# AIflowerQ/InvPref_KDD_2022

Measured on AMD Instinct MI355X. Metric: training interactions/sec, Yahoo-implicit InvPref, higher is better.
Workload: dtype f32; 1 GPU; yahoo_r3_implicit_shaped; users=15400, items=1000, envs=4, factor_num=64, scaling=strong, interactions_total=250154, global_batch=8192, interactions_per_gpu=250154, batch_per_gpu=8192, estep_every_steps=155, parallelism=single GPU

## Files before the change

### invpref_kdd_2022_amd/csrc/invpref_plan.cpp

```cpp
#include "../../include/invpref_plan.h"

#include <algorithm>
#include <atomic>
#include <cstdlib>
#include <cmath>
#include <cstring>
#include <exception>
#include <memory>
#include <mutex>
#include <thread>
#include <vector>

struct InvPrefHostPlan {
    std::vector<int32_t> arr[8];
    std::unique_ptr<int32_t[]> big[8];
    size_t big_n[8] = {0, 0, 0, 0, 0, 0, 0, 0};
    int32_t *alloc(int which, size_t n) {
        big[which].reset(new int32_t[n ? n : 1]);
        big_n[which] = n;
        return big[which].get();
    }
};

namespace {
// ... 263 lines not shown
    for (int c = 0; c < ncls; c++) {
        n_ur[(size_t)c] = (int32_t)cit[(size_t)(2 * c)].size();
        n_ir[(size_t)c] = (int32_t)cit[(size_t)(2 * c + 1)].size();
        uit.insert(uit.end(), cit[(size_t)(2 * c)].begin(), cit[(size_t)(2 * c)].end());
        const std::vector<int32_t> &rows = srows[(size_t)c];
        int64_t k = (int64_t)std::nearbyint(p.stream_split * (double)rows.size());
        if (p.fill_cap) {
            const int64_t room = p.fill_cap / ncls - cdiv(n_ur[(size_t)c], p.rounds_per_task);
            k = std::min<int64_t>((int64_t)rows.size(), std::max<int64_t>(k, room * p.rows_per_stream_task));
        }
        k = std::max<int64_t>(0, std::min<int64_t>(k, (int64_t)rows.size()));
        for (int li = 0; li < 2; li++) {
            const int64_t a = li == 0 ? 0 : k, b = li == 0 ? k : (int64_t)rows.size();
            std::vector<int32_t> &dst = li == 0 ? s1[(size_t)c] : s2[(size_t)c];
            for (int64_t q = a; q < b; q++)
                if (rows[(size_t)q] & kItemBit) dst.push_back(rows[(size_t)q]);
            for (int64_t q = a; q < b; q++)
                if (!(rows[(size_t)q] & kItemBit)) dst.push_back(rows[(size_t)q]);
        }
    }
    for (int c = 0; c < ncls; c++) {
        cls[c][0] = ub; cls[c][1] = n_ur[(size_t)c]; ub += n_ur[(size_t)c];
        cls[c][4] = ib; cls[c][5] = n_ir[(size_t)c]; ib += n_ir[(size_t)c];
    }
    int32_t sb = 0;
    for (int c = 0; c < ncls; c++) { cls[c][2] = sb; cls[c][3] = (int32_t)s1[(size_t)c].size(); sb += cls[c][3]; }
    for (int c = 0; c < ncls; c++) { cls[c][6] = sb; cls[c][7] = (int32_t)s2[(size_t)c].size(); sb += cls[c][7]; }
    {
        std::vector<size_t> off((size_t)(2 * ncls));
        size_t tot[2] = {0, 0};
        for (int q = 0; q < 2 * ncls; q++) { off[(size_t)q] = tot[q & 1]; tot[q & 1] += cd[(size_t)q].size(); }
        int32_t *const dst[2] = {hp->alloc(0, tot[0]), hp->alloc(1, tot[1])};
        parallel_for(2 * ncls, nt, [&](int q) {
            if (!cd[(size_t)q].empty()) std::memcpy(dst[q & 1] + off[(size_t)q], cd[(size_t)q].data(), cd[(size_t)q].size() * 4);
            std::vector<int32_t>().swap(cd[(size_t)q]);
        });
    }
    for (int c = 0; c < ncls; c++) sr.insert(sr.end(), s1[(size_t)c].begin(), s1[(size_t)c].end());
    for (int c = 0; c < ncls; c++) sr.insert(sr.end(), s2[(size_t)c].begin(), s2[(size_t)c].end());
    hp->arr[7].assign(&cls[0][0], &cls[0][0] + 64);
    return hp;
}

InvPrefHostPlan *build_alt(const int64_t *cu, const int64_t *ci, const float *cy, int64_t n, const int64_t *pu, const int64_t *pi,
                           int64_t n_prev, int64_t U, int64_t I, const InvPrefAltPlanParams &p) {
    const bool has_cur = n > 0, has_prev = pu != nullptr && n_prev >= 0;
    if (U <= 0 || I <= 0 || n < 0 || (p.side != 0 && p.side != 1) || p.per_slice < 1 || p.n_classes < 1 || p.n_classes > 8 ||
        p.pend_job_min < 1 || p.pend_per_slice < 1 || (p.slots != 16 && p.slots != 32) || (has_cur && (!cu || !ci || !cy)) || (has_prev && (!pu || !pi)))
        return nullptr;
    const int ng = p.slots;
    const int ncls = p.n_classes;
    const int64_t own_num = p.side == 0 ? U : I, oth_num = p.side == 0 ? I : U;
    const int64_t *own = p.side == 0 ? cu : ci, *oth = p.side == 0 ? ci : cu, *ownp = p.side == 0 ? pu : pi;
    InvPrefHostPlan *hp = new InvPrefHostPlan();
    std::vector<int32_t> &lst = hp->arr[2], &ps = hp->arr[3];
    Side S, T, Sp;
    lst.assign((size_t)n * 4, 0);
    ps.assign((size_t)n, 0);
    bool ok = sort_side(own, n, own_num, S, 1, [&](int64_t i, int64_t j) {
        int32_t *d = lst.data() + (size_t)j * 4;
        d[0] = (int32_t)oth[i];
        d[1] = (int32_t)i;
        std::memcpy(d + 2, cy + i, 4);
    });
    ok = ok && sort_side(oth, n, oth_num, T, 1, [&](int64_t i, int64_t j) { ps[(size_t)i] = (int32_t)j; });
    ok = ok && sort_side(ownp, has_prev ? n_prev : 0, own_num, Sp, 1, [&](int64_t, int64_t) {});
    if (!ok) {
        delete hp;
        return nullptr;
    }
    std::vector<int32_t> &desc = hp->arr[0], &pend = hp->arr[1], &stream = hp->arr[4];
    int32_t cls[8][4];
    std::memset(cls, 0, sizeof(cls));
    int32_t rb = 0;
    std::vector<std::vector<int32_t>> srows((size_t)ncls);
    for (int c = 0; c < ncls; c++) {
        std::vector<int32_t> arows, jrows;
        for (int64_t r = 0; r < own_num; r++) {
            if ((r >> kClassShift) % ncls != c) continue;
            if (S.cnt[(size_t)r] > 0) arows.push_back((int32_t)r);
            else if (Sp.cnt[(size_t)r] >= p.pend_job_min) jrows.push_back((int32_t)r);
            else srows[(size_t)c].push_back((int32_t)r);
        }
        std::vector<int32_t> d, it;
        if (has_cur) side_rounds(S, n, lst.data(), 4, 3, ng, p.per_slice, 1, 2, arows, d, it);
        const size_t n_a = d.size() / ((size_t)ng * 8);
        if (!jrows.empty()) side_rounds(Sp, 0, nullptr, 0, 0, ng, p.pend_per_slice, 1, 0, jrows, d, it);
        const size_t nr = d.size() / ((size_t)ng * 8);
        const size_t pbase = pend.size();
        pend.resize(pbase + nr * ng * 4, 0);
        for (size_t r = 0; r < nr; r++) {
            bool any = false;
            for (int sl = 0; sl < ng; sl++) {
                int32_t *dd = d.data() + (r * ng + sl) * 8, *pp = pend.data() + pbase + (r * ng + sl) * 4;
                const int64_t row = dd[0];
                if (row < 0) continue;
                const int gf = (dd[1] >> 1) & 31, g = gf ? gf : 32, k = sl % g;
                const int64_t cp = Sp.cnt[(size_t)row], p0 = Sp.ptr[(size_t)row];
                const int64_t ln = cdiv(cp, g);
                pp[0] = (int32_t)(p0 + std::min<int64_t>(k * ln, cp));
                pp[1] = (int32_t)(p0 + std::min<int64_t>((k + 1) * ln, cp));
                pp[2] = (int32_t)cp;
                any = any || cp > 0;
                if (r >= n_a) {
                    dd[1] &= 0x3f;
                    for (int q = 2; q < 8; q++) dd[q] = 0;
                }
            }
            if (any)
                for (int sl = 0; sl < ng; sl++) d[(r * ng + sl) * 8 + 1] |= (int32_t)0x80000000u;
        }
        desc.insert(desc.end(), d.begin(), d.end());
        cls[c][0] = rb;
        cls[c][1] = (int32_t)nr;
        rb += (int32_t)nr;
    }
    int32_t sb = 0;
    for (int c = 0; c < ncls; c++) {
        cls[c][2] = sb;
        cls[c][3] = (int32_t)srows[(size_t)c].size();
        sb += cls[c][3];
        for (int32_t r : srows[(size_t)c]) {
            const int32_t e[4] = {r, (int32_t)Sp.ptr[(size_t)r], (int32_t)Sp.ptr[(size_t)r + 1], (int32_t)Sp.cnt[(size_t)r]};
            stream.insert(stream.end(), e, e + 4);
        }
    }
    hp->arr[5].assign(&cls[0][0], &cls[0][0] + 32);
    return hp;
}

}

extern "C" {

static InvPrefHostPlan *build_alt_guarded(const int64_t *cu, const int64_t *ci, const float *cy, int64_t n, const int64_t *pu,
                                          const int64_t *pi, int64_t n_prev, int64_t U, int64_t I, const InvPrefAltPlanParams *p) {
    if (!p) return nullptr;
    try {
        return build_alt(cu, ci, cy, n, pu, pi, n_prev, U, I, *p);
    } catch (...) {
        return nullptr;
    }
}

InvPrefHostPlan *invpref_alt_plan_build(const int64_t *cur_users, const int64_t *cur_items, const float *cur_scores, int64_t n,
                                        const int64_t *prev_users, const int64_t *prev_items, int64_t n_prev,
                                        int64_t user_num, int64_t item_num, const InvPrefAltPlanParams *params) {
    return build_alt_guarded(cur_users, cur_items, cur_scores, n, prev_users, prev_items, n_prev, user_num, item_num, params);
}

int invpref_alt_plan_build_many(const int64_t *users, const int64_t *items, const float *scores, const int64_t *cur_lo,
                                const int64_t *cur_n, const int64_t *prev_lo, const int64_t *prev_n, const int32_t *side,
                                int32_t count, int64_t user_num, int64_t item_num, const InvPrefAltPlanParams *params,
                                InvPrefHostPlan **out, int32_t n_threads) {
    if (!users || !items || !scores || !cur_lo || !cur_n || !prev_lo || !prev_n || !side || !params || !out || count < 0) return -1;
    int nt = n_threads > 0 ? n_threads : (int)std::min<unsigned>(kMaxThreads, std::max(1u, std::thread::hardware_concurrency()));
    nt = std::max(1, std::min(nt, (int)count));
    std::atomic<int> next{0};
    auto work = [&]() {
        for (;;) {
            const int k = next.fetch_add(1);
            if (k >= count) return;
            InvPrefAltPlanParams p = *params;
            p.side = side[k];
            const bool hp = prev_n[k] >= 0;
            out[k] = build_alt_guarded(users + cur_lo[k], items + cur_lo[k], scores + cur_lo[k], cur_n[k],
// ... 100 lines not shown
```

### invpref_kdd_2022_amd/csrc/step_alt.hpp

```cpp

#ifdef ALT_STAMPS
#define ASTAMP(i) STAMP(i)
#else
#define ASTAMP(i) do { } while (0)
#endif

struct AltArgs {
    float *own_p[2];
    float *own_m[2], *own_v[2];
    const float *oth_p[2];
    float *Ev, *W, *b;
    float *mEv, *mW, *mb, *vEv, *vW, *vb;
    int E, D;
    const int4 *desc;
    const int4 *pend;
    const int4 *list;
    const int *push_slot;
    const int4 *stream;
    int rounds_per_task, rows_per_stream_task, n_cls;
    int cls[8][4];
    const int64_t *envs;
    const float *weights;
    StepScalars k;
    float r2_prev, r1_prev;
// ... 122 lines not shown
    if (lane < EMAX) scw[lane] = x.cw;
}
__device__ __forceinline__ void alt_stage_plain(const AltArgs &a, float *sEv, float *sW, float *sb, float *scw, bool pure) {
    constexpr int EMAX = 4, DP = 64;
    const int lane = threadIdx.x & 63;
    bool on[4], onb;
    alt_stage_lanes(a, lane, on, onb);
#pragma unroll
    for (int i = 0; i < 4; i++) {
        const int idx = lane + 64 * i, e = idx / DP, d = idx - e * DP;
        const bool o = on[i] && !pure;
        sEv[idx] = o ? a.Ev[e * a.D + d] : 0.f;
        sW[idx] = o ? a.W[e * a.D + d] : 0.f;
    }
    if (lane < EMAX) sb[lane] = (onb && !pure) ? a.b[lane] : 0.f;
    if (lane < EMAX) scw[lane] = ((a.flags & INVPREF_WEIGHTS_BY_ENV) && onb && !pure) ? a.weights[lane] : 1.f;
}

template <int THREADS>
struct AltGeo {
    static constexpr int NG = THREADS / 16, WAVES = THREADS / 64, DP = 64, EMAX = 4;
    static constexpr int SLAB = 2 * EMAX * DP + EMAX + kLossSlots;
    static constexpr int sEv = 0, sW = sEv + EMAX * DP, sb = sW + EMAX * DP;
    static constexpr int scw = sb + EMAX;
    static constexpr int mv = scw + EMAX;
    static constexpr int red = mv + WAVES * 4 * 64 * 4;
    static constexpr int total = red + NG * SLAB;
};

__device__ __forceinline__ void adam4_prev(float4 &p, float4 g, float4 &m, float4 &v, const AdamScalars &ad, float2 prev2) {
    AdamScalars ap = ad;
    ap.step_size = prev2.x; ap.bc2_sqrt = prev2.y;
    adam4(p, g, m, v, ap);
}

template <bool VEC, bool FULL, int MODE, int THREADS>
__device__ __forceinline__ void alt_task(const AltArgs &a, int r0, int slab_index, float *lds,
                                         const AdamScalars &ad_cur, float2 prev2, const StepScalars &k, int gen) {
    constexpr int LG = 16, EMAX = 4, UE = 2;
    using G = AltGeo<THREADS>;
    using L = AltGeo<THREADS>;
    static_assert(EvalLds<16, 4>::total == AltGeo<256>::total, "alt_task: the smallest-instance layout");
    constexpr int NG = G::NG, DP = G::DP;
    float *sEv = lds + L::sEv, *sW = lds + L::sW, *sb = lds + L::sb, *scw = lds + L::scw;
    float4 *mv = reinterpret_cast<float4 *>(lds + L::mv);
    float *red = lds + L::red;
    const int lg = threadIdx.x & (LG - 1), grp = threadIdx.x / LG, wave = threadIdx.x >> 6, lane = threadIdx.x & 63;
    float4 *mv_wave = mv + wave * 4 * 64;
    const bool implicit = a.flags & INVPREF_IMPLICIT;
    const bool rw_rec = a.flags & INVPREF_REWEIGHT_REC, rw_cls = a.flags & INVPREF_REWEIGHT_CLS;
    const bool by_env = a.flags & INVPREF_WEIGHTS_BY_ENV;
    const bool reg_env = a.flags & INVPREF_REG_ENV_EMBED;
    const bool pure = a.flags & INVPREF_PURE_MF;
    const bool dense = (a.flags & INVPREF_DENSE_REG) && !(a.flags & INVPREF_REG_ONLY_EMBED) && !pure;
    constexpr bool has_prev = MODE & 1, has_cur = MODE & 2;
    const int D = a.D;
    float *own0 = a.own_p[0], *own1 = a.own_p[1];
    const float *oth0 = a.oth_p[0], *oth1 = a.oth_p[1];

    ASTAMP(0);
    int4 d = a.desc[(r0 * NG + grp) * 2], d1 = a.desc[(r0 * NG + grp) * 2 + 1];
    int4 pd = make_int4(0, 0, 0, 0);
    if (has_prev) pd = a.pend[r0 * NG + grp];
    ASTAMP(1);
    float accLi = 0.f, accLe = 0.f, accLc = 0.f, accL2 = 0.f, accL1 = 0.f;
    float *slab = a.slabs + (int64_t)slab_index * G::SLAB;
    auto slot_of = [&](int g) {
        constexpr int GW = 64 / LG;
        return lds + L::mv + (g / GW) * (4 * 64 * 4) + (g % GW) * 2 * DP;
    };

    {
        constexpr int nr = 1;
        const int r = r0;
        const int4 dd = d, dd1 = d1;
        const int4 pdd = pd;
        const int row = dd.x, meta = dd.y;
        const bool active = row >= 0, leader = meta & 1;
        const int slices_f = (meta >> 1) & 31, mode = (meta >> 6) & 7;
        const int slices = slices_f ? slices_f : 32;
        const bool rpend = has_prev && (meta < 0);
        const int cnt_i = (meta >> 9) & 0x3fffff;
        const int nsmp = (active && has_cur) ? (mode == 7 ? dd.w - dd.z : mode) : 0;
        if (r == r0 + STAMP_ROUND) ASTAMP(2);
        const int s_lo = dd.z, s_hi1 = max(dd.w - 1, dd.z);
        const int *dwords = reinterpret_cast<const int *>(a.desc + (r * NG + grp) * 2);
        auto sample_at = [&](int sidx) {
            USample sm;
            if (FULL) {
                const int *src = mode == 7 ? reinterpret_cast<const int *>(a.list + min(s_lo + sidx, s_hi1)) : dwords + 2 + 3 * min(sidx, 1);
                sm.oth = src[0]; sm.ps = src[1]; sm.y = __builtin_bit_cast(float, src[2]);
            } else if (mode == 7) {
                const int4 q = a.list[dd.z + sidx];
                sm.oth = q.x; sm.ps = q.y; sm.y = __builtin_bit_cast(float, q.z);
            } else if (sidx == 0) { sm.oth = dd.z; sm.ps = dd.w; sm.y = __builtin_bit_cast(float, dd1.x); }
            else { sm.oth = dd1.y; sm.ps = dd1.z; sm.y = __builtin_bit_cast(float, dd1.w); }
            return sm;
        };
        const int rowc = active ? row : 0;
        float4 oi = row4<VEC, FULL>(own0, rowc, D, lg), oe = f4zero();
        float4 mi = row4<VEC, FULL>(a.own_m[0], rowc, D, lg), vi = row4<VEC, FULL>(a.own_v[0], rowc, D, lg);
        float4 me = f4zero(), ve = f4zero();
        if (!pure) {
            oe = row4<VEC, FULL>(own1, rowc, D, lg);
            me = row4<VEC, FULL>(a.own_m[1], rowc, D, lg); ve = row4<VEC, FULL>(a.own_v[1], rowc, D, lg);
        }
        constexpr int PB = kAltPendBatch;
        static_assert(PB * 2 * 64 * 4 <= 4 * G::SLAB && (4 * G::SLAB) % 4 == 0 && G::red % 4 == 0, "landing block: the wave's four slab rows");
        const int npend = (active && has_prev) ? pdd.y - pdd.x : 0;
        const float *pbase = a.pend_rows + (unsigned)(npend > 0 ? pdd.x : 0) * (unsigned)(2 * DP) + lg * 4;
        float *land = red + wave * 4 * G::SLAB;
        auto pland = [&](int s0) {
#pragma unroll
            for (int j = 0; j < PB; j++) {
                if (s0 + j < npend) {
                    const float *p = pbase + (unsigned)(s0 + j) * (unsigned)(2 * DP);
                    __builtin_amdgcn_global_load_lds((const __attribute__((address_space(1))) void *)p,
                                                     (__attribute__((address_space(3))) void *)(land + (2 * j) * 256), 16, 0, 0);
                    if (!pure)
                        __builtin_amdgcn_global_load_lds((const __attribute__((address_space(1))) void *)(p + DP),
                                                         (__attribute__((address_space(3))) void *)(land + (2 * j + 1) * 256), 16, 0, 0);
                }
            }
        };
        float4 gpi = f4zero(), gpe = f4zero();
        int n_wave = 0;
        if (rpend) {
            n_wave = npend;
#pragma unroll
            for (int g = 0; g < 64 / LG; g++) n_wave = max(n_wave, __builtin_amdgcn_readlane(npend, g * LG));
            pland(0);
        }

        struct Slot {
            float4 qi, qa;
            USample sm;
            int e, cs;
            float w;
        };
        Slot sl[UE];
        USample idn[UE];
        auto gather = [&](Slot &q, const USample &sm) {
            q.sm = sm;
            q.qi = row4<VEC, FULL>(oth0, sm.oth, D, lg);
            if (FULL) {
                const unsigned pso = (unsigned)sm.ps;
                if (!pure) {
                    q.qa = row4<VEC, FULL>(oth1, sm.oth, D, lg);
                    q.e = *reinterpret_cast<const int *>(reinterpret_cast<const char *>(a.envs) + pso * 8u);
                }
                if ((rw_rec || rw_cls) && !by_env) q.w = *reinterpret_cast<const float *>(reinterpret_cast<const char *>(a.weights) + pso * 4u);
                q.cs = *reinterpret_cast<const int *>(reinterpret_cast<const char *>(a.push_slot) + pso * 4u);
                return;
            }
            if (!pure) {
                q.qa = row4<VEC, FULL>(oth1, sm.oth, D, lg);
                q.e = (int)a.envs[sm.ps];
            }
            if ((rw_rec || rw_cls) && !by_env) q.w = a.weights[sm.ps];
            q.cs = a.push_slot[sm.ps];
        };
#pragma unroll
        for (int j = 0; j < UE; j++) {
            sl[j].qi = sl[j].qa = f4zero();
            sl[j].sm = USample{0, 0, 0.f};
            sl[j].e = sl[j].cs = 0;
            sl[j].w = 1.f;
            idn[j] = USample{0, 0, 0.f};
        }
        USample ls[2 * UE];
#pragma unroll
        for (int j = 0; j < 2 * UE; j++) ls[j] = USample{0, 0, 0.f};
        if (has_cur) {
            if (FULL) {
                if (__builtin_amdgcn_ballot_w64(mode == 7) != 0) {
#pragma unroll
                    for (int j = 0; j < 2 * UE; j++) {
                        const int4 q = a.list[mode == 7 ? min(s_lo + j, s_hi1) : 0];
                        ls[j] = USample{q.x, q.y, __builtin_bit_cast(float, q.z)};
                    }
                }
            } else {
#pragma unroll
                for (int j = 0; j < 2 * UE; j++)
                    if (j < nsmp) ls[j] = sample_at(j);
            }
        }
        auto psum = [&](int s0) {
            asm volatile("s_waitcnt vmcnt(0)" ::: "memory");
            float4 xi[PB], xe[PB];
#pragma unroll
            for (int j = 0; j < PB; j++) {
                xi[j] = *reinterpret_cast<const float4 *>(land + (2 * j) * 256 + lane * 4);
                xe[j] = pure ? f4zero() : *reinterpret_cast<const float4 *>(land + (2 * j + 1) * 256 + lane * 4);
            }
#pragma unroll
            for (int j = 0; j < PB; j++) {
                const bool has = s0 + j < npend;
                f4add(gpi, has ? xi[j] : f4zero());
                if (!pure) f4add(gpe, has ? xe[j] : f4zero());
            }
            if (s0 + PB < n_wave) pland(s0 + PB);
        };
        if (n_wave > 0) psum(0);
        if (has_cur) {
#pragma unroll
            for (int j = 0; j < UE; j++) {
                if (FULL) {
                    USample sm = ls[j];
                    if (mode != 7) sm = j == 0 ? USample{dd.z, dd.w, __builtin_bit_cast(float, dd1.x)} : USample{dd1.y, dd1.z, __builtin_bit_cast(float, dd1.w)};
                    if (mode == 0 || !active) sm = USample{0, 0, 0.f};
                    gather(sl[j], sm);
                } else if (j < nsmp) {
                    gather(sl[j], ls[j]);
                }
                idn[j] = ls[UE + j];
            }
        }
        AltStage stg;
#pragma unroll
        for (int i = 0; i < 9; i++) stg.g[i] = 0ull;
        stg.cw = 1.f;
        if (has_prev) {
            if (rpend) {
                for (int s0 = PB; s0 < n_wave; s0 += PB) psum(s0);
                if (slices > 1) {
                    float *mine = slot_of(grp);
                    *reinterpret_cast<float4 *>(mine + lg * 4) = gpi;
                    *reinterpret_cast<float4 *>(mine + DP + lg * 4) = gpe;
                    __syncthreads();
                    const int lead = grp & ~(slices - 1);
                    if (VEC && slices >= 8) {
                        if (active && leader) {
                            gpi = gpe = f4zero();
#pragma nounroll
                            for (int s = 0; s < slices; s += 8) {
                                float4 xi[8], xe[8];
                                const float *s8 = slot_of(lead + s) + lg * 4;
#pragma unroll
                                for (int j = 0; j < 8; j++) {
                                    xi[j] = *reinterpret_cast<const float4 *>(s8 + (j / 4) * (4 * 64 * 4) + (j % 4) * 2 * DP);
                                    xe[j] = *reinterpret_cast<const float4 *>(s8 + (j / 4) * (4 * 64 * 4) + (j % 4) * 2 * DP + DP);
                                }
#pragma unroll
                                for (int j = 0; j < 8; j++) { f4add(gpi, xi[j]); f4add(gpe, xe[j]); }
                            }
                            *reinterpret_cast<float4 *>(mine + lg * 4) = gpi;
                            *reinterpret_cast<float4 *>(mine + DP + lg * 4) = gpe;
                        }
                        __syncthreads();
                        gpi = *reinterpret_cast<const float4 *>(slot_of(lead) + lg * 4);
                        gpe = *reinterpret_cast<const float4 *>(slot_of(lead) + DP + lg * 4);
                    } else if (VEC && slices == 4) {
                        float4 xi[4], xe[4];
#pragma unroll
                        for (int j = 0; j < 4; j++) {
                            xi[j] = *reinterpret_cast<const float4 *>(slot_of(lead + j) + lg * 4);
                            xe[j] = *reinterpret_cast<const float4 *>(slot_of(lead + j) + DP + lg * 4);
                        }
                        gpi = gpe = f4zero();
#pragma unroll
                        for (int j = 0; j < 4; j++) { f4add(gpi, xi[j]); f4add(gpe, xe[j]); }
                    } else {
                        gpi = gpe = f4zero();
#pragma nounroll
                        for (int s = 0; s < slices; s++) {
                            f4add(gpi, *reinterpret_cast<const float4 *>(slot_of(lead + s) + lg * 4));
                            f4add(gpe, *reinterpret_cast<const float4 *>(slot_of(lead + s) + DP + lg * 4));
                        }
                    }
                    __syncthreads();
                }
            }
            const float cp = (float)pdd.z;
            if (cp != 0.f) {
                f4fma(gpi, cp, reg_term(oi, a.r2_prev, a.r1_prev));
                f4fma(gpe, cp, reg_term(oe, a.r2_prev, a.r1_prev));
            }
            adam4_prev(oi, gpi, mi, vi, ad_cur, prev2);
            if (!pure) adam4_prev(oe, gpe, me, ve, ad_cur, prev2);
        }
        if (r == r0 + STAMP_ROUND) ASTAMP(3);
        if (!has_cur) {
            if (active && leader) {
                put4<VEC, 0, FULL>(own0, row, D, lg, oi);
                put4<VEC, 0, FULL>(a.own_m[0], row, D, lg, mi);
                put4<VEC, 0, FULL>(a.own_v[0], row, D, lg, vi);
                if (!pure) {
                    put4<VEC, 0, FULL>(own1, row, D, lg, oe);
                    put4<VEC, 0, FULL>(a.own_m[1], row, D, lg, me);
                    put4<VEC, 0, FULL>(a.own_v[1], row, D, lg, ve);
                }
            }
            return;
        }
        mv_wave[0 * 64 + lane] = mi; mv_wave[1 * 64 + lane] = vi;
        if (!pure) { mv_wave[2 * 64 + lane] = me; mv_wave[3 * 64 + lane] = ve; }
        if (r == r0) {
            {
                constexpr int ZR4 = (2 * EMAX * DP + EMAX) / 4;
                static_assert((2 * EMAX * DP + EMAX) % 4 == 0 && G::SLAB % 4 == 0, "16-byte zeroing");
#pragma unroll
                for (int t = 0; t < (4 * ZR4 + 63) / 64; t++) {
                    const int i = lane + 64 * t;
                    if (i < 4 * ZR4) *reinterpret_cast<float4 *>(land + (i / ZR4) * G::SLAB + (i % ZR4) * 4) = f4zero();
                }
            }
            if (wave == 0) {
                if (has_prev && !pure) alt_stage_issue(a, stg);
                if (has_prev && !pure) alt_stage_finish(a, stg, gen, sEv, sW, sb, scw);
                else alt_stage_plain(a, sEv, sW, sb, scw, pure);
            }
            __syncthreads();
            ASTAMP(4);
        }
        float4 gi = f4zero(), ge = f4zero();
        auto step = [&](const Slot &q, bool has) {
            const int e = q.e;
            if (has) {
                const float wq = by_env ? scw[e] : q.w;
                const float w_rec = rw_rec ? wq : 1.f, w_cls = rw_cls ? wq : 1.f;
                const float4 ev = *reinterpret_cast<const float4 *>(sEv + e * DP + lg * 4);
                Eval<EMAX> o;
                eval_interaction<LG, EMAX>(o, oi, q.qi, oe, q.qa, ev, sW, sb, nullptr, a.E, e, q.sm.y, w_rec * k.invB,
                                           w_cls * k.invB, k, implicit, pure, lg);
                float4 gip;
                gip.x = o.g_p - k.alpha * o.gx.x; gip.y = o.g_p - k.alpha * o.gx.y;
                gip.z = o.g_p - k.alpha * o.gx.z; gip.w = o.g_p - k.alpha * o.gx.w;
                f4add(gi, f4mul(gip, q.qi));
                f4fma(ge, o.g_q, f4mul(q.qa, ev));
                float *cr = a.push_rows + (unsigned)q.cs * (unsigned)(2 * DP) + lg * 4;
                store4<kAltPushSt>(cr, f4mul(gip, oi));
                store4<kAltPushSt>(cr + DP, f4scale(o.g_q, f4mul(oe, ev)));
                float4 oo = f4scale(o.g_q, f4mul(oe, q.qa));
                if (reg_env) f4add(oo, reg_term(ev, 2.f * k.r2, 2.f * k.r1));
                float *mine = red + grp * G::SLAB;
#pragma unroll
                for (int c = 0; c < EMAX; c++) {
                    float4 *wr = reinterpret_cast<float4 *>(mine + EMAX * DP + c * DP + lg * 4);
                    float4 cur = *wr;
                    f4fma(cur, o.gz[c], o.x);
                    *wr = cur;
                }
                if (lg == 0) {
                    float4 *br = reinterpret_cast<float4 *>(mine + 2 * EMAX * DP);
                    float4 cur = *br;
                    cur.x += o.gz[0]; cur.y += o.gz[1]; cur.z += o.gz[2]; cur.w += o.gz[3];
                    *br = cur;
                }
                float4 *erow = reinterpret_cast<float4 *>(mine + e * DP + lg * 4);
                float4 cur = *erow;
                f4add(cur, oo);
                *erow = cur;
                float s2a = 0.f, s2b = 0.f;
                sq_acc(s2a, s2b, q.qi);
                sq_acc(s2a, s2b, q.qa);
                float s2 = s2a + s2b, s1 = abs_acc(abs_acc(0.f, q.qi), q.qa);
                if (reg_env) { s2 += 2.f * f4sq(ev); s1 += 2.f * f4abs(ev); }
                accL2 += s2;
                accL1 += s1;
                if (lg == 0) { accLi += o.li * w_rec; accLe += o.le * w_rec; }
                if (lg == 0) accLc += o.lcls * w_cls;
            }
        };
        for (int s = 0; s < nsmp; s += UE) {
#pragma unroll
            for (int j = 0; j < UE; j++) {
                if (s + j < nsmp) step(sl[j], true);
                if (FULL || s + UE + j < nsmp) gather(sl[j], idn[j]);
                if (FULL || s + 2 * UE + j < nsmp) idn[j] = sample_at(s + 2 * UE + j);
            }
        }
        if (r == r0 + STAMP_ROUND) ASTAMP(5);
        const float cnt = (float)cnt_i;
        if (active && leader) {
            accL2 += cnt * (f4sq(oi) + f4sq(oe));
            accL1 += cnt * (f4abs(oi) + f4abs(oe));
        }
        const bool last = r == r0 + nr - 1;
        if (last) {
            accLi = row16_sum(accLi); accLe = row16_sum(accLe); accLc = row16_sum(accLc);
            accL2 = row16_sum(accL2); accL1 = row16_sum(accL1);
            if (lg == 0) {
                float *ls = red + grp * G::SLAB + 2 * EMAX * DP + EMAX;
                ls[0] = accLi; ls[1] = accLe; ls[2] = accLc; ls[3] = accL2; ls[4] = accL1;
                ls[5] = ls[6] = ls[7] = 0.f;
            }
            if (dense && slab_index == 0 && wave == 0) {
                const float4 w4 = *reinterpret_cast<const float4 *>(sW + lane * 4);
                float w2 = f4sq(w4), w1 = f4abs(w4);
                const float bb = lane < EMAX ? sb[lane] : 0.f;
                float b2 = bb * bb, b1 = fabsf(bb);
                w2 = wave_sum_valu(w2); w1 = wave_sum_valu(w1); b2 = wave_sum_valu(b2); b1 = wave_sum_valu(b1);
                if (lane == 0) {
                    float *ls = red + 2 * EMAX * DP + EMAX;
                    ls[5] = w2 / ((float)a.D * (float)a.E) + b2 / (float)a.E;
                    ls[6] = w1 / ((float)a.D * (float)a.E) + b1 / (float)a.E;
                }
            }
        }
        if (active && leader) {
            mi = mv_wave[0 * 64 + lane]; vi = mv_wave[1 * 64 + lane];
            if (!pure) { me = mv_wave[2 * 64 + lane]; ve = mv_wave[3 * 64 + lane]; }
        }
        asm volatile("" ::: "memory");
        if (slices > 1) {
            float *mine = slot_of(grp);
            *reinterpret_cast<float4 *>(mine + lg * 4) = gi;
            *reinterpret_cast<float4 *>(mine + DP + lg * 4) = ge;
        }
        if (slices > 1 || last) __syncthreads();
        if (last) {
            static_assert(G::SLAB % 4 == 0 && G::SLAB / 4 <= THREADS && NG % 8 == 0, "slab sum: one float4 column set per thread");
            if ((int)threadIdx.x < G::SLAB / 4) {
                const float *col = red + threadIdx.x * 4;
                float4 sum = *reinterpret_cast<const float4 *>(col);
#pragma unroll
                for (int q0 = 0; q0 < NG; q0 += 8) {
                    float4 x[8];
#pragma unroll
                    for (int j = 0; j < 8; j++) x[j] = *reinterpret_cast<const float4 *>(col + (q0 + j) * G::SLAB);
#pragma unroll
                    for (int j = (q0 == 0 ? 1 : 0); j < 8; j++) f4add(sum, x[j]);
                }
                store4<kAltSlabSt>(slab + threadIdx.x * 4, sum);
            }
        }
        if (slices > 1) {
            if (active && leader) {
                if (VEC && slices >= 8) {
                    float4 xi[8], xe[8];
#pragma unroll
                    for (int j = 1; j < 8; j++) {
                        xi[j] = *reinterpret_cast<const float4 *>(slot_of(grp + j) + lg * 4);
                        xe[j] = *reinterpret_cast<const float4 *>(slot_of(grp + j) + DP + lg * 4);
                    }
#pragma unroll
                    for (int j = 1; j < 8; j++) { f4add(gi, xi[j]); f4add(ge, xe[j]); }
#pragma nounroll
                    for (int s = 8; s < slices; s += 8) {
#pragma unroll
                        for (int j = 0; j < 8; j++) {
                            xi[j] = *reinterpret_cast<const float4 *>(slot_of(grp + s + j) + lg * 4);
                            xe[j] = *reinterpret_cast<const float4 *>(slot_of(grp + s + j) + DP + lg * 4);
                        }
#pragma unroll
                        for (int j = 0; j < 8; j++) { f4add(gi, xi[j]); f4add(ge, xe[j]); }
                    }
                } else if (VEC && slices == 4) {
                    float4 xi[4], xe[4];
#pragma unroll
                    for (int j = 1; j < 4; j++) {
                        xi[j] = *reinterpret_cast<const float4 *>(slot_of(grp + j) + lg * 4);
// ... 411 lines not shown
```

### invpref_kdd_2022_amd/plan.py

```python
from __future__ import annotations

import ctypes as C
import os
from dataclasses import dataclass

import numpy as np
import torch

THREADS = 256
ITEM_BIT = 1 << 30
MODE_LIST = 7
MAX_ROW_COUNT = 1 << 22
TARGET_WORKGROUPS = 1536
RESIDENT_SMALL = 768


class RowPlanStruct(C.Structure):
    _fields_ = [('n', C.c_int32), ('lanes_per_group', C.c_int32), ('n_user_rounds', C.c_int32),
                ('n_item_rounds', C.c_int32), ('user_rounds_per_task', C.c_int32), ('item_rounds_per_task', C.c_int32),
                ('user_desc', C.c_void_p), ('item_desc', C.c_void_p), ('user_round_iters', C.c_void_p),
                ('user_list', C.c_void_p), ('item_list', C.c_void_p), ('n_stream', C.c_int32),
                ('rows_per_stream_task', C.c_int32), ('stream_rows', C.c_void_p), ('n_classes', C.c_int32),
                ('rows_per_stream_task2', C.c_int32), ('cls', C.c_int32 * 64), ('push_slot', C.c_void_p),
                ('rec_slot', C.c_void_p)]
# ... 549 lines not shown
        cu, ci = (np.ascontiguousarray(cur[0], np.int64), np.ascontiguousarray(cur[1], np.int64)) if has_cur else (z64, z64)
        cy = np.ascontiguousarray(cur[2], np.float32) if has_cur else np.zeros(0, np.float32)
        pu, pi = (np.ascontiguousarray(prev[0], np.int64), np.ascontiguousarray(prev[1], np.int64)) if has_prev else (z64, z64)
        ps = AltPlanParamsStruct(side, per_slice, n_classes, ALT_PEND_JOB_MIN, ALT_PEND_PER_SLICE, slots)
        h = L.invpref_alt_plan_build(cu.ctypes.data, ci.ctypes.data, cy.ctypes.data, len(cu),
                                     pu.ctypes.data if has_prev else None, pi.ctypes.data if has_prev else None, len(pu),
                                     user_num, item_num, C.byref(ps))
        if not h:
            raise ValueError('native alt plan builder: invalid arguments (row ids out of range?)')
        return _alt_from_handle(L, h, side, has_prev, has_cur, len(cu), len(pu), per_slice, n_classes, rows_per_stream_task,
                                n_partials_prev, slots)
    if has_cur:
        u, i, y = (np.asarray(cur[0], np.int64), np.asarray(cur[1], np.int64), np.asarray(cur[2], np.float32))
        own, oth = (u, i) if side == 0 else (i, u)
        n = len(own)
        po = np.argsort(own, kind='stable')
        cols = (oth[po].astype(np.int32), po.astype(np.int32), y.view(np.int32)[po])
        own_sorted = own[po]
        cnt = np.bincount(own, minlength=own_num).astype(np.int64)
        push_slot = np.argsort(np.argsort(oth, kind='stable'), kind='stable').astype(np.int32)
        lst = np.stack([cols[0], cols[1], cols[2], np.zeros(n, np.int32)], axis=1).reshape(-1)
    else:
        n = 0
        cols, own_sorted = (np.zeros(0, np.int32),) * 3, np.zeros(0, np.int64)
        cnt = np.zeros(own_num, np.int64)
        push_slot, lst = np.zeros(0, np.int32), np.zeros(0, np.int32)
    if has_prev:
        ownp = np.asarray(prev[0] if side == 0 else prev[1], np.int64)
        n_prev = len(ownp)
        cntp = np.bincount(ownp, minlength=own_num).astype(np.int64)
    else:
        n_prev = 0
        cntp = np.zeros(own_num, np.int64)
    if n and max(cnt.max(), cntp.max()) >= MAX_ROW_COUNT:
        raise ValueError('a row with too many interactions in one minibatch overflows the job descriptor')
    ptrp = np.concatenate([[0], np.cumsum(cntp)])
    pjob = (cnt == 0) & (cntp >= ALT_PEND_JOB_MIN)
    rcls = row_class(np.arange(own_num), n_classes)
    d_parts, p_parts, s_parts = [], [], []
    cls = np.zeros((8, 4), np.int32)
    ownp_sorted = np.sort(ownp, kind='stable') if has_prev else np.zeros(0, np.int64)
    for c in range(n_classes):
        parts = []
        if has_cur:
            d, _ = _side_rounds(own_sorted, cols, own_num, ng, per_slice, 1, 2, skip=(cnt == 0) | (rcls != c))
            parts.append(d)
        if pjob.any():
            d, _ = _side_rounds(ownp_sorted, (), own_num, ng, ALT_PEND_PER_SLICE, 1, 0, skip=~pjob | (rcls != c))
            parts.append(d)
        d = np.concatenate(parts) if parts else np.zeros((0, ng, 8), np.int32)
        d = d[(d[:, :, 0] >= 0).any(axis=1)] if len(d) else d
        pend = np.zeros((len(d), ng, 4), np.int32)
        if len(d):
            row = d[:, :, 0].astype(np.int64)
            act = row >= 0
            rowc = np.where(act, row, 0)
            g = (d[:, :, 1] >> 1) & 31
            g = np.where(g == 0, 32, g)
            k = np.arange(ng)[None, :] % np.maximum(g, 1)
            cp = np.where(act, cntp[rowc], 0)
            ln = -(-cp // np.maximum(g, 1))
            a0 = ptrp[rowc] + np.minimum(k * ln, cp)
            b0 = ptrp[rowc] + np.minimum((k + 1) * ln, cp)
            pend_only = act & (cnt[rowc] == 0)
            pend[:, :, 0] = np.where(act, a0, 0)
            pend[:, :, 1] = np.where(act, b0, 0)
            pend[:, :, 2] = cp
            meta = d[:, :, 1]
            meta = np.where(pend_only, meta & 0x3f, meta)
            d[:, :, 1] = meta
            d[:, :, 2:] = np.where(pend_only[:, :, None], 0, d[:, :, 2:])
            has = (cp > 0).any(axis=1)
            d[:, :, 1] |= np.where(has, np.int32(-2 ** 31), np.int32(0))[:, None]
        pad = (-len(d)) % rounds_per_task
        if pad:
            idle = np.zeros((pad, ng, 8), np.int32)
            idle[:, :, 0] = -1
            idle[:, :, 1] = 1 << 1
            d = np.concatenate([d, idle])
            pend = np.concatenate([pend, np.zeros((pad, ng, 4), np.int32)])
        d_parts.append(d)
        p_parts.append(pend)
        rows = np.flatnonzero((cnt == 0) & ~pjob & (rcls == c))
        s = np.stack([rows, ptrp[rows], ptrp[rows + 1], cntp[rows]], axis=1).astype(np.int32)
        s_parts.append(s)
    rb = sb = 0
    for c in range(n_classes):
        cls[c] = rb, len(d_parts[c]), sb, len(s_parts[c])
        rb += len(d_parts[c])
        sb += len(s_parts[c])
    desc = np.concatenate(d_parts)
    return dict(side=side, has_prev=int(has_prev), has_cur=int(has_cur), n=n, n_prev=n_prev, lanes_per_group=lanes,
                slots_per_round=ng, rounds_per_task=rounds_per_task, desc=desc, pend=np.concatenate(p_parts), list=lst, push_slot=push_slot,
                stream=np.concatenate(s_parts).reshape(-1), n_stream=sb, rows_per_stream_task=rows_per_stream_task,
                n_classes=n_classes, cls=cls, n_partials_prev=int(n_partials_prev),
                n_tasks=(len(desc) // rounds_per_task if has_cur else 0), per_slice=per_slice)


def _alt_from_handle(L, h, side, has_prev, has_cur, n, n_prev, per_slice, n_classes, rows_per_stream_task, n_partials_prev,
                     slots=16) -> dict:
    out = []
    try:
        for which in range(6):
            ptr = C.POINTER(C.c_int32)()
            ln = L.invpref_plan_array(h, which, C.byref(ptr))
            out.append(np.ctypeslib.as_array(ptr, shape=(ln,)).copy() if ln > 0 else np.zeros(0, np.int32))
    finally:
        L.invpref_plan_free(h)
    desc, pend, lst, push_slot, stream, cls = out
    desc = desc.reshape(-1, slots, 8)
    return dict(side=side, has_prev=int(has_prev), has_cur=int(has_cur), n=int(n), n_prev=int(n_prev), lanes_per_group=16,
                slots_per_round=slots, rounds_per_task=1, desc=desc, pend=pend.reshape(-1, slots, 4), list=lst, push_slot=push_slot, stream=stream,
                n_stream=len(stream) // 4, rows_per_stream_task=rows_per_stream_task, n_classes=n_classes,
                cls=cls.reshape(8, 4).copy(), n_partials_prev=int(n_partials_prev), n_tasks=(len(desc) if has_cur else 0),
                per_slice=per_slice)


def alt_slots_for(own_rows: np.ndarray, n_rows: int, per_slice: int, n_classes: int = N_CLASSES) -> int:
    cnt = np.bincount(np.asarray(own_rows, np.int64), minlength=n_rows)
    c = cnt[cnt > 0]
    if len(c) == 0:
        return 16
    need = np.maximum(1, -(-c // per_slice))
    slices = np.minimum(32, 1 << np.ceil(np.log2(need)).astype(np.int64))
    rounds = sum(-(-int((slices == g).sum()) // (32 // g)) for g in (1, 2, 4, 8, 16, 32))
    rounds += n_classes * len(np.unique(slices)) // 2
    return 32 if rounds + 48 <= 256 else 16


def build_alt_plans(users: np.ndarray, items: np.ndarray, scores: np.ndarray, specs, user_num: int, item_num: int,
                    factor_num: int = 64, per_slice_u: int | None = None, per_slice_i: int | None = None,
                    n_classes: int | None = None, rows_per_stream_task: int | None = None, threads: int = 0,
                    slots_u: int = 16, slots_i: int = 16) -> list:
    users, items = np.ascontiguousarray(users, np.int64), np.ascontiguousarray(items, np.int64)
    scores = np.ascontiguousarray(scores, np.float32)
    if per_slice_u is None:
        per_slice_u = ALT_PER_SLICE
    if per_slice_i is None:
        per_slice_i = ALT_PER_SLICE
    if n_classes is None:
        n_classes = N_CLASSES
    n_classes = max(1, min(8, n_classes))
    if rows_per_stream_task is None:
        rows_per_stream_task = stream_rows_default(factor_num)

    def rng(r):
        return None if r is None else (users[r[0]:r[0] + r[1]], items[r[0]:r[0] + r[1]], scores[r[0]:r[0] + r[1]])
    L = _native_lib()
    if L is not None and (per_slice_u != per_slice_i or slots_u != slots_i):
        out = [None] * len(specs)
        for sd in (0, 1):
            idx = [j for j, sp in enumerate(specs) if sp[2] == sd]
            if idx:
                ps, sl = (per_slice_i, slots_i) if sd else (per_slice_u, slots_u)
                for j, pl in zip(idx, build_alt_plans(users, items, scores, [specs[j] for j in idx], user_num, item_num,
                                                      factor_num=factor_num, per_slice_u=ps, per_slice_i=ps, n_classes=n_classes,
                                                      rows_per_stream_task=rows_per_stream_task, threads=threads, slots_u=sl,
                                                      slots_i=sl)):
                    out[j] = pl
        return out
    if L is None:
        return [build_alt_plan(rng(c), None if pv is None else rng(pv)[:2], side, user_num, item_num, factor_num=factor_num,
                               per_slice=per_slice_i if side else per_slice_u, n_classes=n_classes,
                               rows_per_stream_task=rows_per_stream_task, slots=slots_i if side else slots_u)
                for c, pv, side in specs]
    k = len(specs)
# ... 99 lines not shown
```

Measured before the change: 527.9 million interactions/s.

## Bound FULL-mode sample loop by wave max count and skip idle-wave loads

In FULL mode, the per-round sample loop and the gathers now run only up to the wave-wide maximum sample count, where before they walked the full padded count. Own-row parameter and Adam state loads are skipped when no lane in the wave is active, and list prefetches past the wave maximum are skipped. Streaming rows are reordered so rows with pending work come first, in both the C++ and Python planners, which groups idle rows together. The change adds readlane and ballot reductions, explicit tail handling for leftover samples, and compiler barriers that pin registers. The risk is divergence or correctness bugs in the tail path.

Measured after the change: 538.9 million interactions/s (median of 6 runs). 1.02x the previous value.

```diff
diff --git a/invpref_kdd_2022_amd/csrc/invpref_plan.cpp b/invpref_kdd_2022_amd/csrc/invpref_plan.cpp
--- a/invpref_kdd_2022_amd/csrc/invpref_plan.cpp
+++ b/invpref_kdd_2022_amd/csrc/invpref_plan.cpp
@@ -369,6 +369,7 @@
             else if (Sp.cnt[(size_t)r] >= p.pend_job_min) jrows.push_back((int32_t)r);
             else srows[(size_t)c].push_back((int32_t)r);
         }
+        std::stable_partition(srows[(size_t)c].begin(), srows[(size_t)c].end(), [&](int32_t r) { return Sp.cnt[(size_t)r] > 0; });
         std::vector<int32_t> d, it;
         if (has_cur) side_rounds(S, n, lst.data(), 4, 3, ng, p.per_slice, 1, 2, arows, d, it);
         const size_t n_a = d.size() / ((size_t)ng * 8);
diff --git a/invpref_kdd_2022_amd/csrc/step_alt.hpp b/invpref_kdd_2022_amd/csrc/step_alt.hpp
--- a/invpref_kdd_2022_amd/csrc/step_alt.hpp
+++ b/invpref_kdd_2022_amd/csrc/step_alt.hpp
@@ -228,6 +228,11 @@
         const bool rpend = has_prev && (meta < 0);
         const int cnt_i = (meta >> 9) & 0x3fffff;
         const int nsmp = (active && has_cur) ? (mode == 7 ? dd.w - dd.z : mode) : 0;
+        int w_n = 0;
+#pragma unroll
+        for (int g = 0; g < 64 / LG; g++) w_n = max(w_n, __builtin_amdgcn_readlane(nsmp, g * LG));
+        const bool w_act = __builtin_amdgcn_ballot_w64(active) != 0;
+        asm volatile("" : "+v"(d1.x), "+v"(d1.y), "+v"(d1.z), "+v"(d1.w));
         if (r == r0 + STAMP_ROUND) ASTAMP(2);
         const int s_lo = dd.z, s_hi1 = max(dd.w - 1, dd.z);
         const int *dwords = reinterpret_cast<const int *>(a.desc + (r * NG + grp) * 2);
@@ -243,17 +248,24 @@
             else { sm.oth = dd1.y; sm.ps = dd1.z; sm.y = __builtin_bit_cast(float, dd1.w); }
             return sm;
         };
+        const int npend = (active && has_prev) ? pdd.y - pdd.x : 0;
+        int n_wave = 0;
+        if (rpend) {
+#pragma unroll
+            for (int g = 0; g < 64 / LG; g++) n_wave = max(n_wave, __builtin_amdgcn_readlane(npend, g * LG));
+        }
         const int rowc = active ? row : 0;
-        float4 oi = row4<VEC, FULL>(own0, rowc, D, lg), oe = f4zero();
-        float4 mi = row4<VEC, FULL>(a.own_m[0], rowc, D, lg), vi = row4<VEC, FULL>(a.own_v[0], rowc, D, lg);
-        float4 me = f4zero(), ve = f4zero();
-        if (!pure) {
-            oe = row4<VEC, FULL>(own1, rowc, D, lg);
-            me = row4<VEC, FULL>(a.own_m[1], rowc, D, lg); ve = row4<VEC, FULL>(a.own_v[1], rowc, D, lg);
+        float4 oi = f4zero(), oe = f4zero(), mi = f4zero(), vi = f4zero(), me = f4zero(), ve = f4zero();
+        if (w_act) {
+            oi = row4<VEC, FULL>(own0, rowc, D, lg);
+            mi = row4<VEC, FULL>(a.own_m[0], rowc, D, lg); vi = row4<VEC, FULL>(a.own_v[0], rowc, D, lg);
+            if (!pure) {
+                oe = row4<VEC, FULL>(own1, rowc, D, lg);
+                me = row4<VEC, FULL>(a.own_m[1], rowc, D, lg); ve = row4<VEC, FULL>(a.own_v[1], rowc, D, lg);
+            }
         }
         constexpr int PB = kAltPendBatch;
         static_assert(PB * 2 * 64 * 4 <= 4 * G::SLAB && (4 * G::SLAB) % 4 == 0 && G::red % 4 == 0, "landing block: the wave's four slab rows");
-        const int npend = (active && has_prev) ? pdd.y - pdd.x : 0;
         const float *pbase = a.pend_rows + (unsigned)(npend > 0 ? pdd.x : 0) * (unsigned)(2 * DP) + lg * 4;
         float *land = red + wave * 4 * G::SLAB;
         auto pland = [&](int s0) {
@@ -270,13 +282,7 @@
             }
         };
         float4 gpi = f4zero(), gpe = f4zero();
-        int n_wave = 0;
-        if (rpend) {
-            n_wave = npend;
-#pragma unroll
-            for (int g = 0; g < 64 / LG; g++) n_wave = max(n_wave, __builtin_amdgcn_readlane(npend, g * LG));
-            pland(0);
-        }
+        if (rpend) pland(0);
 
         struct Slot {
             float4 qi, qa;
@@ -322,9 +328,13 @@
                 if (__builtin_amdgcn_ballot_w64(mode == 7) != 0) {
 #pragma unroll
                     for (int j = 0; j < 2 * UE; j++) {
-                        const int4 q = a.list[mode == 7 ? min(s_lo + j, s_hi1) : 0];
-                        ls[j] = USample{q.x, q.y, __builtin_bit_cast(float, q.z)};
+                        if (j < 3 || w_n > j) {
+                            const int4 q = a.list[mode == 7 ? min(s_lo + j, s_hi1) : 0];
+                            ls[j] = USample{q.x, q.y, __builtin_bit_cast(float, q.z)};
+                        }
                     }
+#pragma unroll
+                    for (int j = 0; j < 2 * UE; j++) asm volatile("" : "+v"(ls[j].oth), "+v"(ls[j].ps), "+v"(ls[j].y));
                 }
             } else {
 #pragma unroll
@@ -350,18 +360,26 @@
         };
         if (n_wave > 0) psum(0);
         if (has_cur) {
-#pragma unroll
-            for (int j = 0; j < UE; j++) {
-                if (FULL) {
-                    USample sm = ls[j];
-                    if (mode != 7) sm = j == 0 ? USample{dd.z, dd.w, __builtin_bit_cast(float, dd1.x)} : USample{dd1.y, dd1.z, __builtin_bit_cast(float, dd1.w)};
-                    if (mode == 0 || !active) sm = USample{0, 0, 0.f};
-                    gather(sl[j], sm);
-                } else if (j < nsmp) {
-                    gather(sl[j], ls[j]);
-                }
-                idn[j] = ls[UE + j];
-            }
+            static_assert(UE == 2, "the nested form below: two slots");
+            if (FULL) {
+                USample sm0 = ls[0], sm1 = ls[1];
+                if (mode != 7) {
+                    sm0 = USample{d.z, d.w, __builtin_bit_cast(float, d1.x)};
+                    sm1 = USample{d1.y, d1.z, __builtin_bit_cast(float, d1.w)};
+                }
+                if (mode == 0 || !active) sm0 = sm1 = USample{0, 0, 0.f};
+                asm volatile("" : "+v"(sm0.oth), "+v"(sm0.ps), "+v"(sm0.y), "+v"(sm1.oth), "+v"(sm1.ps), "+v"(sm1.y));
+                if (w_n > 0) {
+                    gather(sl[0], sm0);
+                    if (w_n > 1) gather(sl[1], sm1);
+                }
+            } else {
+#pragma unroll
+                for (int j = 0; j < UE; j++)
+                    if (j < nsmp) gather(sl[j], ls[j]);
+            }
+#pragma unroll
+            for (int j = 0; j < UE; j++) idn[j] = ls[UE + j];
         }
         AltStage stg;
 #pragma unroll
@@ -509,12 +527,35 @@
                 if (lg == 0) accLc += o.lcls * w_cls;
             }
         };
-        for (int s = 0; s < nsmp; s += UE) {
-#pragma unroll
-            for (int j = 0; j < UE; j++) {
-                if (s + j < nsmp) step(sl[j], true);
-                if (FULL || s + UE + j < nsmp) gather(sl[j], idn[j]);
-                if (FULL || s + 2 * UE + j < nsmp) idn[j] = sample_at(s + 2 * UE + j);
+        if (FULL) {
+            static_assert(UE == 2, "the tail below: two slots");
+            int s = 0;
+            for (; s + 2 * UE <= w_n; s += UE) {
+#pragma unroll
+                for (int j = 0; j < UE; j++) {
+                    if (s + j < nsmp) step(sl[j], true);
+                    gather(sl[j], idn[j]);
+                    idn[j] = sample_at(s + 2 * UE + j);
+                }
+            }
+            const int rest = w_n - s;
+            if (rest == 3) {
+                if (s < nsmp) step(sl[0], true);
+                gather(sl[0], idn[0]);
+                if (s + 1 < nsmp) step(sl[1], true);
+                if (s + 2 < nsmp) step(sl[0], true);
+            } else if (rest > 0) {
+                if (s < nsmp) step(sl[0], true);
+                if (rest == 2 && s + 1 < nsmp) step(sl[1], true);
+            }
+        } else {
+            for (int s = 0; s < nsmp; s += UE) {
+#pragma unroll
+                for (int j = 0; j < UE; j++) {
+                    if (s + j < nsmp) step(sl[j], true);
+                    if (s + UE + j < nsmp) gather(sl[j], idn[j]);
+                    if (s + 2 * UE + j < nsmp) idn[j] = sample_at(s + 2 * UE + j);
+                }
             }
         }
         if (r == r0 + STAMP_ROUND) ASTAMP(5);
diff --git a/invpref_kdd_2022_amd/plan.py b/invpref_kdd_2022_amd/plan.py
--- a/invpref_kdd_2022_amd/plan.py
+++ b/invpref_kdd_2022_amd/plan.py
@@ -655,6 +655,7 @@
         d_parts.append(d)
         p_parts.append(pend)
         rows = np.flatnonzero((cnt == 0) & ~pjob & (rcls == c))
+        rows = rows[np.argsort(cntp[rows] == 0, kind='stable')]
         s = np.stack([rows, ptrp[rows], ptrp[rows + 1], cntp[rows]], axis=1).astype(np.int32)
         s_parts.append(s)
     rb = sb = 0
```
